# arangesh/Ground-Plane-Polling

Hardware: AMD Instinct MI355X
Metric: images/sec end-to-end (resnet50, 1k planes, 1242x375) (higher is better)
Workload: dtype f16x3

## Files before the change

ground-plane-polling_amd/csrc/decode.hip:

```cpp

#include <hip/hip_runtime.h>
#include <stdint.h>
#include <limits.h>

#include <atomic>
#include <mutex>
#include <vector>

#include "gpp.h"

namespace {

constexpr int kCounterStride = 4096;
constexpr int kHeaderBytes = 64 * kCounterStride;
constexpr int kKeptCountWord = 1;
constexpr int kKeptKeysOffset = 1024;

__device__ __forceinline__ float cephes_expf(float x)
{
    x = fminf(fmaxf(x, -88.3762626647949f), 88.3762626647949f);
    float fx = floorf(x * 1.44269504088896341f + 0.5f);
    x = (x - fx * 0.693359375f) - fx * -2.12194440e-4f;
    const float z = x * x;
    float y = 1.9875691500e-4f;
// ... 766 lines not shown
}

__global__ __launch_bounds__(kCompactThreads) void compact_pixels_kernel(uint32_t* __restrict__ bitmap, const LevelTable T, int B, int max_rows,
                                                                         int32_t* __restrict__ rows, int32_t* __restrict__ counts,
                                                                         int32_t* __restrict__ flag, const int32_t* __restrict__ or_flag)
{
    compact_pixels(bitmap, T, B, max_rows, rows, counts, flag, or_flag);
}

struct CompactJob { uint32_t* bitmap; int32_t* rows; int32_t* counts; int32_t* flag; const int32_t* or_flag; };
__global__ __launch_bounds__(kCompactThreads) void compact_pixels_pair_kernel(const CompactJob a, const CompactJob b, const CompactJob c, const LevelTable T,
                                                                              int B, int max_rows)
{
    const CompactJob& j = blockIdx.x == 0 ? a : blockIdx.x == 1 ? b : c;
    compact_pixels(j.bitmap, T, B, max_rows, j.rows, j.counts, j.flag, j.or_flag);
}

__global__ __launch_bounds__(256) void mark_candidate_pixels_kernel(const float* __restrict__ cls, int64_t n_anchors, int nba, float thr,
                                                                    const LevelTable T, int B, int total_words, uint32_t* __restrict__ marks)
{
    __shared__ unsigned long long hit[4];
    const int lane = threadIdx.x & 63, wave = threadIdx.x >> 6;
    const int64_t gbit0 = (int64_t)blockIdx.x * 256 + wave * 64;
    const int word0 = (int)(gbit0 >> 5);
    if (lane == 0) hit[wave] = 0;
    __syncthreads();
    for (int i = 0; i < nba; ++i) {
        const int j = i * 64 + lane, q = j / nba, k = j - q * nba;
        const int word = word0 + (q >> 5);
        if (word >= total_words) continue;
// ... 79 lines not shown
#pragma unroll
        for (int s = 32; s >= 1; s >>= 1) n[k] += __shfl_down(n[k], s, 64);
        if (lane == 0) sums[k][wave] = n[k];
    }
    __syncthreads();
    if (tid == 0) {
        int t[4] = {0, 0, 0, 0};
        for (int q = 0; q < kCompactThreads / 64; ++q) { t[0] += sums[0][q]; t[1] += sums[1][q]; t[2] += sums[2][q]; t[3] += sums[3][q]; }
        const int f3 = (t[0] > max_rows || t[1] > tower_max_rows) ? 1 : 0;
        const int f2 = (f3 || t[2] > deep_max_rows) ? 1 : 0;
        stats[0] = t[0];
        stats[1] = t[1];
        stats[2] = f3;
        stats[3] = f2;
        if (stats0 != nullptr) stats0[0] = (f2 || t[3] > deep_max_rows) ? 1 : 0;
    }
}

std::mutex g_deep_mutex;
std::vector<gpp_deep_list_desc> g_deep_descs;
std::vector<char> g_deep_held;

}

extern "C" int gpp_detect_pixel_lists(const gpp_pixel_list_desc* host_desc, void* stream)
{
    if (!host_desc) return GPP_ERR_BAD_ARG;
    const gpp_pixel_list_desc& d = *host_desc;
    if (d.B < 0 || d.B > kMaxBatch || d.n_anchors <= 0 || d.n_anchors > kMaxAnchors || d.num_base_anchors <= 0 || d.max_rows < 0 ||
        d.n_levels < 1 || d.n_levels > GPP_MAX_GROUPS || (d.lists_per_image != 1 && d.lists_per_image != 4) || d.reserved != 0 || d.reserved2 != 0)
// ... 45 lines not shown

int deep_lists_table(const gpp_deep_list_desc& d, LevelTable& T, int64_t& words)
{
    if (d.B < 0 || d.B > kMaxBatch || d.n_anchors <= 0 || d.n_anchors > kMaxAnchors || d.num_base_anchors <= 0 || d.num_base_anchors > 64 ||
        d.max_rows < 0 || d.tower_max_rows < 0 || d.deep_max_rows < 0 || d.n_levels < 1 || d.n_levels > GPP_MAX_GROUPS || d.reserved != 0 ||
        !(d.score_thr == d.score_thr))
        return GPP_ERR_BAD_ARG;
    const bool layer1 = d.rows1 || d.counts1 || d.flag1;
    const bool layer0 = d.radius4 || d.rows0 || d.counts0 || d.flag0 || d.stats0;
    if (layer0 && (!d.radius4 || !d.rows0 || !d.counts0 || !d.flag0 || !d.stats0 || !d.rows1 || !d.counts1 || !d.flag1)) return GPP_ERR_BAD_ARG;
    if (d.B > 0 && (!d.cls_logits || !d.marks || !d.radius1 || !d.radius2 || !d.radius3 || !d.rows2 || !d.counts2 || !d.flag2 || !d.stats ||
                    (layer1 && (!d.rows1 || !d.counts1 || !d.flag1))))
        return GPP_ERR_BAD_ARG;
    if (((uintptr_t)d.cls_logits & 15) || (((uintptr_t)d.marks | (uintptr_t)d.radius1 | (uintptr_t)d.radius2 | (uintptr_t)d.radius3 | (uintptr_t)d.rows2 |
          (uintptr_t)d.counts2 | (uintptr_t)d.flag2 | (uintptr_t)d.rows1 | (uintptr_t)d.counts1 | (uintptr_t)d.flag1 | (uintptr_t)d.stats |
          (uintptr_t)d.radius4 | (uintptr_t)d.rows0 | (uintptr_t)d.counts0 | (uintptr_t)d.flag0 | (uintptr_t)d.stats0) & 3))
        return GPP_ERR_ALIGN;
    T.n_levels = d.n_levels;
    int64_t pixels = 0;
    words = 0;
    for (int l = 0; l < GPP_MAX_GROUPS; ++l) {
        const int pix = l < d.n_levels ? d.level_pixels[l] : 0;
        if (l < d.n_levels && pix <= 0) return GPP_ERR_BAD_ARG;
        if ((int64_t)d.B * (pixels + pix) >= (1LL << 31)) return GPP_ERR_UNSUPPORTED;
        T.pix[l] = pix;
        T.pix_begin[l] = (int)pixels;
        T.word_begin[l] = (int)words;
        T.list_begin[l] = (int)((int64_t)d.B * pixels);
        T.width[l] = l < d.n_levels ? d.level_width[l] : 0;
        if (l < d.n_levels && (T.width[l] <= 0 || pix % T.width[l] != 0)) return GPP_ERR_BAD_ARG;
        pixels += pix;
        words += ((int64_t)d.B * pix + 31) / 32;
    }
    if (pixels * d.num_base_anchors != d.n_anchors) return GPP_ERR_BAD_ARG;
    return GPP_OK;
}

}

extern "C" int gpp_detect_deep_lists(const gpp_deep_list_desc* host_desc, void* stream)
{
    if (!host_desc) return GPP_ERR_BAD_ARG;
    const gpp_deep_list_desc& d = *host_desc;
    LevelTable T;
    int64_t words = 0;
    const int rc = deep_lists_table(d, T, words);
    if (rc != GPP_OK) return rc;
    if (d.B == 0) return GPP_OK;
    hipStream_t st = (hipStream_t)stream;
    const unsigned blocks = (unsigned)(((words + 1) / 2 * 64 + 255) / 256);
    mark_candidate_pixels_kernel<<<dim3(blocks), 256, 0, st>>>(d.cls_logits, d.n_anchors, d.num_base_anchors, d.score_thr, T, d.B, (int)words, d.marks);
    if (d.radius4) dilate_radii_kernel<true><<<dim3(blocks), 256, 0, st>>>(d.marks, T, d.B, (int)words, d.radius1, d.radius2, d.radius3, d.radius4);
    else dilate_radii_kernel<false><<<dim3(blocks), 256, 0, st>>>(d.marks, T, d.B, (int)words, d.radius1, d.radius2, d.radius3, nullptr);
    deep_stats_kernel<<<1, kCompactThreads, 0, st>>>(d.marks, d.radius1, d.radius2, (int)words, d.max_rows, d.tower_max_rows, d.deep_max_rows, d.stats,
                                                     d.radius3, d.stats0);
    const CompactJob layer2 = {d.radius2, d.rows2, d.counts2, d.flag2, d.stats + 2}, layer1 = {d.radius3, d.rows1, d.counts1, d.flag1, d.stats + 3};
    const CompactJob layer0 = {d.radius4, d.rows0, d.counts0, d.flag0, d.stats0};
    if (d.rows1) compact_pixels_pair_kernel<<<d.rows0 ? 3 : 2, kCompactThreads, 0, st>>>(layer2, layer1, layer0, T, d.B, d.deep_max_rows);
    else compact_pixels_kernel<<<1, kCompactThreads, 0, st>>>(d.radius2, T, d.B, d.deep_max_rows, d.rows2, d.counts2, d.flag2, d.stats + 2);
    const hipError_t e = hipGetLastError();
    return e == hipSuccess ? GPP_OK : (int)e;
}

extern "C" int gpp_detect_deep_lists_register(const gpp_deep_list_desc* host_desc, int32_t* handle)
{
    if (!host_desc || !handle) return GPP_ERR_BAD_ARG;
    LevelTable T;
    int64_t words = 0;
// ... 81 lines not shown
```

ground-plane-polling_amd/keras_retinanet_3D/backend/hip.py:

```python

import ctypes
import os

_LIB = None
_HERE = os.path.dirname(os.path.abspath(__file__))
LIB_PATH = os.environ.get('GPP_LIB') or os.path.normpath(os.path.join(_HERE, '..', '..', 'lib', 'libgpp_hip.so'))
CSRC_DIR = os.path.normpath(os.path.join(_HERE, '..', '..', 'csrc'))

GPP_OK = 0
_ERRORS = {
    -1: 'GPP_ERR_BAD_ARG',
    -2: 'GPP_ERR_WORKSPACE',
    -3: 'GPP_ERR_ALIGN',
    -4: 'GPP_ERR_UNSUPPORTED',
}

c_void_p = ctypes.c_void_p
c_int = ctypes.c_int
c_float = ctypes.c_float
c_size_t = ctypes.c_size_t
c_int64 = ctypes.c_int64


GPP_BF16 = 1
# ... 52 lines not shown
class PixelListDesc(ctypes.Structure):
    _fields_ = [('workspace', c_void_p), ('bitmap', c_void_p), ('rows', c_void_p), ('counts', c_void_p), ('flag', c_void_p),
                ('n_anchors', c_int64)] + \
               [(n, ctypes.c_int32) for n in ('B', 'num_base_anchors', 'lists_per_image', 'n_levels', 'max_rows', 'reserved')] + \
               [('level_pixels', ctypes.c_int32 * GPP_MAX_GROUPS), ('reserved2', ctypes.c_int32)] + \
               [('dilated_bitmap', c_void_p), ('dilated_rows', c_void_p), ('dilated_counts', c_void_p), ('dilated_flag', c_void_p),
                ('level_width', ctypes.c_int32 * GPP_MAX_GROUPS), ('dilated_max_rows', ctypes.c_int32)]


class DeepListDesc(ctypes.Structure):
    _fields_ = [(n, c_void_p) for n in ('cls_logits', 'marks', 'radius1', 'radius2', 'radius3', 'rows2', 'counts2', 'flag2',
                                        'rows1', 'counts1', 'flag1', 'stats')] + [('n_anchors', c_int64)] + \
               [(n, ctypes.c_int32) for n in ('B', 'num_base_anchors', 'n_levels', 'max_rows', 'tower_max_rows', 'deep_max_rows')] + \
               [('score_thr', c_float), ('reserved', ctypes.c_int32),
                ('level_pixels', ctypes.c_int32 * GPP_MAX_GROUPS), ('level_width', ctypes.c_int32 * GPP_MAX_GROUPS)] + \
               [(n, c_void_p) for n in ('radius4', 'rows0', 'counts0', 'flag0', 'stats0')]


class MobileNetBlockDesc(ctypes.Structure):
    _fields_ = [('inp', c_void_p), ('dw_weight', c_void_p), ('dw_bias', c_void_p), ('pw_weight', c_void_p), ('pw_bias', c_void_p),
                ('out_scale', c_void_p), ('out', c_void_p)] + \
               [(n, ctypes.c_int32) for n in ('dtype', 'B', 'H', 'W', 'C_in', 'C_out', 'stride', 'in_pitch', 'out_pitch', 'weight_rows',
                                              'tile_hint', 'reserved')]


class MobileNetStemDesc(ctypes.Structure):
    _fields_ = [('inp', c_void_p), ('weight', c_void_p), ('bias', c_void_p), ('out', c_void_p)] + \
               [(n, ctypes.c_int32) for n in ('B', 'H', 'W', 'C_out', 'out_pitch', 'reserved')]


class AbsmaxDesc(ctypes.Structure):
# ... 144 lines not shown
        lib.gpp_road_peel_workspace_bytes.argtypes = [c_int, c_int, ctypes.POINTER(c_size_t)]
        lib.gpp_road_peel_i32.restype = c_int
        lib.gpp_road_peel_i32.argtypes = [c_void_p] * 4 + [c_uint32, c_void_p] + [c_int] * 4 + [c_double] + [c_void_p] * 3 + [c_size_t, c_void_p]
    if hasattr(lib, 'gpp_detect_pixel_lists'):
        lib.gpp_detect_pixel_lists.restype = c_int
        lib.gpp_detect_pixel_lists.argtypes = [ctypes.POINTER(PixelListDesc), c_void_p]
    if hasattr(lib, 'gpp_detect_deep_lists'):
        lib.gpp_detect_deep_lists.restype = c_int
        lib.gpp_detect_deep_lists.argtypes = [ctypes.POINTER(DeepListDesc), c_void_p]
        lib.gpp_detect_deep_lists_register.restype = c_int
        lib.gpp_detect_deep_lists_register.argtypes = [ctypes.POINTER(DeepListDesc), ctypes.POINTER(ctypes.c_int32)]
        lib.gpp_detect_deep_lists_release.restype = c_int
        lib.gpp_detect_deep_lists_release.argtypes = [ctypes.c_int32]
        lib.gpp_detect_deep_lists_run.restype = c_int
        lib.gpp_detect_deep_lists_run.argtypes = [ctypes.c_int32, c_int, c_void_p]
    if hasattr(lib, 'gpp_conv2d_deferred_register'):
        lib.gpp_conv2d_deferred_register.restype = c_int
        lib.gpp_conv2d_deferred_register.argtypes = [ctypes.POINTER(ConvDesc), ctypes.POINTER(ctypes.c_int32)]
        lib.gpp_conv2d_deferred_release.restype = c_int
        lib.gpp_conv2d_deferred_release.argtypes = [ctypes.c_int32]
        lib.gpp_conv2d_deferred_run.restype = c_int
        lib.gpp_conv2d_deferred_run.argtypes = [ctypes.c_int32, c_int, c_void_p]
    lib.gpp_conv2d_igemm.restype = c_int
    lib.gpp_conv2d_igemm.argtypes = [ctypes.POINTER(ConvDesc), c_void_p]
    lib.gpp_stem_conv7x7_bn_relu.restype = c_int
    lib.gpp_stem_conv7x7_bn_relu.argtypes = [c_void_p, c_void_p, c_void_p, c_void_p, c_int, c_int, c_int, c_int, c_void_p]
    lib.gpp_stem_conv7x7_bn_relu_mfma.restype = c_int
    lib.gpp_stem_conv7x7_bn_relu_mfma.argtypes = [c_void_p, c_void_p, c_void_p, c_void_p, c_int, c_int, c_int, c_int, c_void_p]
    lib.gpp_stem_pack_weights_f16.restype = c_int
    lib.gpp_stem_pack_weights_f16.argtypes = [c_void_p, c_void_p, c_size_t]
# ... 694 lines not shown
```

ground-plane-polling_amd/keras_retinanet_3D/models/builder.py:

```python

import ctypes

from ..backend import hip
from ..layers import conv as C
from ..layers import mobilenet as M
from ..layers.filter_detections import MAX_DETECTIONS, NMS_THRESHOLD, SCORE_THRESHOLD
from ..utils import anchors as anchor_utils
from ..utils import cuboid_nms as cuboid_nms_utils
from ..utils.gpp_utils import POLL_THRESHOLD, POSE_SCORE_THRESHOLD
from . import weights as W
from .plan import (BlockDesc, BlockProjDesc, CandidatePixelsDesc, CuboidNmsDesc, DensePoolDesc, DetectDesc, PollDesc, PoolDesc, PoseDesc,
                   PreactDesc, RaggedPoolDesc, RaggedStemDesc, ReluDesc, StemDesc, TailDesc,
                   OP_STEM, OP_MAXPOOL, OP_CONV, OP_RELU, OP_DETECT, OP_POLL, OP_TAIL, OP_BLOCK,
                   OP_DETECT_CANDIDATES, OP_DETECT_SELECT, OP_DETECT_EMIT, OP_DETECT_OSF, OP_STEM_POOL,
                   OP_MAXPOOL_PAD, OP_AVGPOOL, OP_CONV_PREACT, OP_MOBILENET_STEM, OP_MOBILENET_BLOCK, OP_POSE, OP_CUBOID_NMS,
                   OP_ABSMAX, OP_ABSMAX_CLEAR, OP_STEM_RAGGED, OP_STEM_POOL_RAGGED, OP_MAXPOOL_RAGGED, OP_DETECT_CANDIDATE_PIXELS,
                   block_form, head_forms, layer_split, part_of, TOWER_SLICES, TOWER0, TOWER0_SLICE, SparseHeads, Plan)


class PlanBuilder(object):

    def __init__(self, model, B, H, Wd, n_planes, planes_batched, ragged=False):
        torch, dev = model.torch, model.device
        self.model, self.torch, self.device = model, torch, dev
# ... 346 lines not shown
            plan.keep += plan.sparse.tensors()
            if forms.deep_layers:
                plan.sparse.add_deep(self.torch, forms.deep_layers, opts.sparse_deep)
                plan.keep += plan.sparse.deep_tensors()
            if forms.tower0:
                plan.sparse.add_tower0(self.torch)
                plan.keep += plan.sparse.tower0_tensors()
        if forms.tower0:
            self.towers_0_split(P, wide)
        else:
            self.conv(TOWER0, P, wide, 3, pad=(1, 1), relu=True, join=True)
        l_dim, l_cls = (1, 2) if opts.head_lanes else (0, 0)
        towers = {'cls': ('pyramid_classification', 256, 512, 'pyramid_classification', cls_o, 0, l_cls or opts.cls_lane),
                  'reg': ('pyramid_regression', 512, 0, 'pyramid_regression_ops', reg_o, 1, 0, bool(opts.cls_lane)),
                  'dim': ('pyramid_regression_dim', 128, 768, 'pyramid_regression_dim', dim_o, 0, l_dim)}
        if opts.decode_overlap:
            self.tower(forms, wide, *towers['cls'])
            self.decode(OP_DETECT_CANDIDATE_PIXELS if plan.sparse else OP_DETECT_CANDIDATES, 'filtered_detections/candidates',
                        lane=opts.cls_lane or 1)
            self.tower(forms, wide, *towers['reg'])
            self.decode(OP_DETECT_SELECT, 'filtered_detections/select', lane=1, sync=True)
            self.tower(forms, wide, *towers['dim'])
            self.decode(OP_DETECT_EMIT, join=True)
        else:
            for t in ('dim', 'cls', 'reg'):
                self.tower(forms, wide, *towers[t])
            self.decode(OP_DETECT_OSF if m.osf else OP_DETECT, join=True)

    def towers_0_split(self, P, wide):
        m, plan, sp = self.model, self.plan, self.plan.sparse
        wt, bias, (kh, kw, cin, cout) = m.conv_w[TOWER0]
# ... 10 lines not shown
                            out_scale=parts[2] if scale is not None else None)
            if m.dtype == 'f16x3':
                d.range_counter = plan.range_slot.data_ptr()
            return d
        rest = desc(n, cout - n)
        plan.conv_descs.append((rest, 0))
        plan.ws_need[0] = max(plan.ws_need.get(0, 0), C.workspace_bytes(rest))
        first = desc(0, n)
        first.weight_rows = n
        first.deep_rows, first.deep_counts, first.deep_flag = sp.tower0_rows.data_ptr(), sp.tower0_counts.data_ptr(), sp.tower0_flag.data_ptr()
        plan.keep.append(first)
        plan.emit(OP_CONV, rest, TOWER0, list(P), cols(n, cout - n), flops=C.conv_flops(rest) + C.conv_flops(first), join=True, io=(P, wide, None))
        self.tower0 = (first, list(P), cols(0, n))

    def tower(self, forms, wide, prefix, width, c0, out_name, out, tag=0, lane=0, join=False):
        src = [C.FMap(f.buf, f.B, f.H, f.W, width, off=f.off + c0, bstride=f.bstride, pitch=f.pitch, split=f.split, half=f.half) for f in wide]
        regression = out_name == 'pyramid_regression_ops'
        for i in range(1, 4):
            name = '{}_{}'.format(prefix, i)
            _, dst = self.pyramid(width)
            if regression and i == 3 and forms.tower_both:
                self.tower_last(name, src, dst, tag, lane)
            elif regression and 3 - forms.deep_layers <= i < 3:
                self.tower_deep(name, src, dst, tag, lane, 2 - i)
            else:
                self.conv(name, src, dst, 3, pad=(1, 1), relu=True, tag=tag, lane=lane)
            src = dst
        self.out_layer('dense' if lane else forms.outputs[out_name], out_name, src, out, lane, join)

    def tower_last(self, name, src, dst, tag, lane):
        sp = self.plan.sparse
        d = self.desc(name, src, dst, 3, pad=(1, 1), relu=True, lane=lane)
        d.tower_rows, d.tower_counts, d.tower_flag = sp.tower_rows.data_ptr(), sp.tower_counts.data_ptr(), sp.tower_flag.data_ptr()
        self.plan.emit(OP_CONV, d, name, list(src) + [sp.tower_rows, sp.tower_counts, sp.tower_flag], dst, tag=tag, flops=C.conv_flops(d), lane=lane,
                       join=not sp.lists_joined, io=(src, dst, None))
        sp.lists_joined = True
        sp.tower.append(d)

    def tower_deep(self, name, src, dst, tag, lane, which):
        sp = self.plan.sparse
        d = self.desc(name, src, dst, 3, pad=(1, 1), relu=True, lane=lane)
        lists = [sp.deep_rows[which], sp.deep_counts[which], sp.deep_flags[which]]
        d.deep_rows, d.deep_counts, d.deep_flag = [t.data_ptr() for t in lists]
        self.plan.emit(OP_CONV, d, name, list(src) + lists, dst, tag=tag, flops=C.conv_flops(d), lane=lane, io=(src, dst, None))
        sp.deep.append(d)

    def out_layer(self, form, name, src, out, lane, join):
        plan, sp = self.plan, self.plan.sparse
        if form == 'lists_after':
            d = self.desc(name, src, out, 3, pad=(1, 1), out_f32=True, lane=lane)
            d.lists_after = sp.register_deep(sp.deep_desc(plan.cls_logits, plan.n_anchors, anchor_utils.NUM_BASE_ANCHORS, SCORE_THRESHOLD))
            reads, writes = list(src), list(out) + sp.deep_tensors()
            if sp.tower0_rows is not None:
                first, p_maps, slice_maps = self.tower0
                sp.register_tower0(first, d)
                reads, writes = reads + p_maps, writes + slice_maps + sp.tower0_tensors()
            plan.emit(OP_CONV, d, name, reads, writes, flops=C.conv_flops(d), lane=lane, join=join, io=(src, out, None))
            return
        if form == 'dense':
            self.conv(name, src, out, 3, pad=(1, 1), out_f32=True, lane=lane, join=join)
            if sp is not None and join and not lane:
                sp.lists_joined = True
            return
        dense = self.desc(name, src, out, 3, pad=(1, 1), out_f32=True, lane=lane)
        dense.guard, dense.guard_value = sp.flag.data_ptr(), 1
        plan.emit(OP_CONV, dense, name, list(src) + [sp.flag], out, flops=C.conv_flops(dense), lane=lane, join=join or not sp.lists_joined,
                  io=(src, out, None))
        sp.lists_joined = True
        rows = self.desc(name, src, out, 3, pad=(1, 1), out_f32=True, lane=lane)
        rows.gather_rows, rows.gather_counts, rows.split_k = sp.rows.data_ptr(), sp.counts.data_ptr(), 1
        rows.guard, rows.guard_value = sp.flag.data_ptr(), 0
        plan.emit(OP_CONV, rows, name, list(src) + [sp.rows, sp.counts, sp.flag], out, lane=lane, io=(src, out, None))
        sp.dense.append(dense)
        sp.gathered.append(rows)

    def poll(self):
        plan, B, n_planes, torch, dev, D = self.plan, self.B, self.n_planes, self.torch, self.device, MAX_DETECTIONS
        plan.keypoints = torch.empty((B, D, 4, 3), dtype=torch.float32, device=dev)
# ... 118 lines not shown
```

ground-plane-polling_amd/keras_retinanet_3D/models/plan.py:

```python

import collections
import ctypes
import os

import numpy as np

from ..backend import hip
from ..layers import conv as C


class StemDesc(ctypes.Structure):
    _fields_ = [('inp', ctypes.c_void_p), ('weight', ctypes.c_void_p), ('bias', ctypes.c_void_p), ('out', ctypes.c_void_p),
                ('dtype', ctypes.c_int32), ('B', ctypes.c_int32), ('H', ctypes.c_int32), ('W', ctypes.c_int32), ('range_counter', ctypes.c_void_p)]


class PoolDesc(ctypes.Structure):
    _fields_ = [('inp', ctypes.c_void_p), ('out', ctypes.c_void_p), ('dtype', ctypes.c_int32), ('B', ctypes.c_int32),
                ('H', ctypes.c_int32), ('W', ctypes.c_int32), ('C', ctypes.c_int32), ('reserved', ctypes.c_int32)]


class RaggedStemDesc(ctypes.Structure):
    _fields_ = [('stem', StemDesc), ('heights', ctypes.c_void_p), ('Hp', ctypes.c_int32), ('reserved', ctypes.c_int32)]


# ... 69 lines not shown
OP_STEM_POOL = 13
OP_MAXPOOL_PAD, OP_AVGPOOL, OP_CONV_PREACT = 17, 18, 32
OP_MOBILENET_STEM, OP_MOBILENET_BLOCK = 33, 34
OP_POSE = 19
OP_CUBOID_NMS = 20
OP_ABSMAX, OP_ABSMAX_CLEAR = 35, 36
OP_STEM_RAGGED, OP_STEM_POOL_RAGGED, OP_MAXPOOL_RAGGED = 37, 38, 39
OP_DETECT_CANDIDATE_PIXELS = 40
DETECT_OPS = (OP_DETECT, OP_DETECT_CANDIDATES, OP_DETECT_SELECT, OP_DETECT_EMIT, 12, OP_DETECT_CANDIDATE_PIXELS)
OP_JOIN, OP_SYNC = 0x10000, 0x20000


PlanOptions = collections.namedtuple('PlanOptions', 'x3_level fuse_stem_pool stage_chunks half_stages fuse_tail fuse_block fuse_block_proj '
                                                    'fuse_block_inproj fuse_inproj_rounds '
                                                    'br1_lane fpn_lanes p4_lane head_lanes decode_overlap cls_lane autotune tune_key sparse_heads '
                                                    'sparse_tower sparse_tower_rounds sparse_deep sparse_deep_rounds sparse_depth')


def plan_options(model, B):
    env = os.environ.get
    x3 = model.dtype in C.X3_TYPES
    x3_split = env('GPP_X3_SPLIT', '2')
    x3_level = int(x3_split) if x3 else 0
    chunks = env('GPP_STAGE_CHUNKS')
    tail_widths = env('GPP_FUSE_TAIL', '64,128')
    fuse_tail = [int(v) for v in tail_widths.split(',') if v.strip() and int(v) > 0]
    if x3:
        fuse_tail = [v for v in fuse_tail if v == 64] if x3_level >= 2 else []
    elif model.esz == 4:
        fuse_tail = []
    block_widths = env('GPP_FUSE_BLOCK', '64,128')
# ... 17 lines not shown
        fuse_inproj_rounds=float(env('GPP_FUSE_INPROJ_MIN_ROUNDS', FUSE_INPROJ_MIN_ROUNDS)),
        br1_lane=env('GPP_BR1_LANE', '1') != '0',
        fpn_lanes=fpn_lanes,
        p4_lane=1 if (fpn_lanes and env('GPP_P4_LANE', '1') != '0') else 0,
        head_lanes=head_lanes,
        decode_overlap=overlap,
        cls_lane=2 if (overlap and env('GPP_CLS_LANE', '1' if B <= 2 else '0') != '0') else 0,
        autotune=env('GPP_AUTOTUNE', '1') != '0',
        sparse_heads=max(1e-9, float(env('GPP_SPARSE_HEADS_MAX_SHARE', SPARSE_HEADS_MAX_SHARE))) if sparse else 0.0,
        sparse_tower=(max(1e-9, float(env('GPP_SPARSE_TOWER_MAX_SHARE', SPARSE_TOWER_MAX_SHARE)))
                      if (sparse and env('GPP_SPARSE_TOWER', '1') != '0') else 0.0),
        sparse_tower_rounds=float(env('GPP_SPARSE_TOWER_MIN_ROUNDS', SPARSE_TOWER_MIN_ROUNDS)),
        sparse_deep=max(1e-9, float(env('GPP_SPARSE_TOWER_DEEP_MAX_SHARE', SPARSE_TOWER_DEEP_MAX_SHARE))),
        sparse_deep_rounds=float(env('GPP_SPARSE_TOWER_DEEP_MIN_ROUNDS', SPARSE_TOWER_DEEP_MIN_ROUNDS)),
        sparse_depth=int(env('GPP_SPARSE_TOWER_DEPTH', SPARSE_TOWER_DEPTH)),
        tune_key='x3split={};fuse={}/{};plan={}{}'.format(x3_split, tail_widths, block_widths, model.plan_mode,
                                                          C.latency_split_config() if model.plan_mode == 'latency' else '') +
                 (';audit' if model.audit else '') + ('' if inproj else ';inproj=0'))


INPROJ_TILE = (8, 14)
FUSE_INPROJ_MIN_ROUNDS = '1'


def inproj_rounds(images, h, w):
    th, tw = INPROJ_TILE
    return images * (-(-h // th)) * (-(-w // tw)) / (2.0 * COMPUTE_UNITS)


def block_form(opts, width, projection, split_input, halves, join, inproj=None):
    if (projection and inproj is not None and opts.fuse_block_inproj and width == 64 and width in opts.fuse_block and inproj[0] == 1 and
            inproj_rounds(*inproj[1:]) > opts.fuse_inproj_rounds):
        return 'block', 'inproj'
# ... 103 lines not shown
        self.flag = torch.ones((1,), dtype=i32, device=device)
        self.dense, self.gathered = [], []
        self.lists_joined = False
        self.tower, self.tower_max_rows = [], 0
        self.tower_bitmap = self.tower_rows = self.tower_counts = self.tower_flag = self.range_scratch = None
        if tower_share > 0.0:
            self.tower_max_rows = max(0, min(total, int(tower_share * total)))
            self.tower_bitmap = torch.zeros_like(self.bitmap)
            self.tower_rows = torch.zeros_like(self.rows)
            self.tower_counts = torch.zeros_like(self.counts)
            self.tower_flag = torch.ones_like(self.flag)
            self.range_scratch = torch.zeros((1,), dtype=torch.int64, device=device)

        self.deep, self.deep_layers, self.deep_max_rows, self.deep_handle = [], 0, 0, 0
        self.deep_bitmaps = self.deep_rows = self.deep_counts = self.deep_flags = self.deep_stats = None
        self.tower0 = self.tower0_carrier = None
        self.tower0_handle = 0
        self.tower0_bitmap = self.tower0_rows = self.tower0_counts = self.tower0_flag = self.tower0_stats = None

    def add_tower0(self, torch):
        self.tower0_bitmap = torch.zeros_like(self.bitmap)
        self.tower0_rows = torch.zeros_like(self.rows)
        self.tower0_counts = torch.zeros_like(self.counts)
        self.tower0_flag = torch.ones_like(self.flag)
        self.tower0_stats = torch.zeros_like(self.flag)

    def tower0_tensors(self):
        if self.tower0_rows is None:
            return []
        return [self.tower0_bitmap, self.tower0_rows, self.tower0_counts, self.tower0_flag, self.tower0_stats]
# ... 25 lines not shown
    def deep_desc(self, cls_logits, n_anchors, num_base_anchors, score_thr):
        d = hip.DeepListDesc()
        d.cls_logits = cls_logits.data_ptr()
        d.marks, d.radius1, d.radius2, d.radius3 = [t.data_ptr() for t in self.deep_bitmaps]
        d.rows2, d.counts2, d.flag2 = self.deep_rows[0].data_ptr(), self.deep_counts[0].data_ptr(), self.deep_flags[0].data_ptr()
        if self.deep_layers > 1:
            d.rows1, d.counts1, d.flag1 = self.deep_rows[1].data_ptr(), self.deep_counts[1].data_ptr(), self.deep_flags[1].data_ptr()
        d.stats = self.deep_stats.data_ptr()
        if self.tower0_rows is not None:
            d.radius4, d.rows0, d.counts0 = self.tower0_bitmap.data_ptr(), self.tower0_rows.data_ptr(), self.tower0_counts.data_ptr()
            d.flag0, d.stats0 = self.tower0_flag.data_ptr(), self.tower0_stats.data_ptr()
        d.n_anchors, d.B, d.num_base_anchors, d.n_levels = n_anchors, self.B, num_base_anchors, len(self.level_pixels)
        d.max_rows, d.tower_max_rows, d.deep_max_rows, d.score_thr = self.max_rows, self.tower_max_rows, self.deep_max_rows, score_thr
        d.level_pixels = (ctypes.c_int32 * hip.GPP_MAX_GROUPS)(*self.level_pixels)
        d.level_width = (ctypes.c_int32 * hip.GPP_MAX_GROUPS)(*self.level_widths)
        return d

    def register_deep(self, desc):
        handle = ctypes.c_int32(0)
        hip.check(hip.lib().gpp_detect_deep_lists_register(ctypes.byref(desc), ctypes.byref(handle)), 'gpp_detect_deep_lists_register')
        self.deep_handle = int(handle.value)
        return self.deep_handle

    def __del__(self):
        if getattr(self, 'deep_handle', 0):
            try:
                hip.lib().gpp_detect_deep_lists_release(self.deep_handle)
            except Exception:
                pass
            self.deep_handle = 0
# ... 31 lines not shown
        for flag in list(self.deep_flags or ()) + ([self.tower0_flag] if self.tower0_flag is not None else []):
            flag.fill_(1)


class Plan(object):

    def __init__(self):
        self.keep = []
        self.io = {}
        self.io_parts = {}
        self.tuning_parts = {}
        self.ops = []
        self.oracle_names = {}
        self.lanes = []
        self.access = []
        self.atomic = []
        self.wrote = []
        self.op_io = []
        self.audit_table = None
        self.audit_maps = []
        self.audit_unobserved = []
        self.inner = {}
        self.open_lanes = set()
        self.conv_descs = []
        self.ws_need = {}
        self.array = None
        self.flops = 0.0
        self.ragged = False
        self.heights = None
        self.sparse = None
        self.heads_stale = False

    @property
    def regression(self):
        self.complete_heads()
        return self._regression

    @regression.setter
# ... 24 lines not shown
                    setattr(d, field, None)
                setattr(d, tile, 0)
                if scratch and d.range_counter:
                    d.range_counter = sp.range_scratch.data_ptr()
                if sp.tower0 is not None and desc is sp.deep[0]:
                    d.conv_before = sp.tower0_handle
                hip.check(hip.lib().gpp_conv2d_igemm(ctypes.byref(d), hip.stream_ptr()), 'gpp_conv2d_igemm ({})'.format(what))

    def emit(self, kind, desc, name, reads=(), writes=(), tag=0, flops=0.0, lane=0, join=False, sync=False, io=None, inner=(), atomic=()):
        self.keep += list(inner) + [desc]
        if inner:
            self.inner[id(desc)] = tuple(inner)
        self.ops.append((kind, tag, desc, name, flops))
        self.lanes.append((int(lane) << 8) | (OP_JOIN if join else 0) | (OP_SYNC if sync else 0))
        self.access.append((self.spans(reads), self.spans(writes)))
        self.atomic.append(self.spans(atomic))
        self.wrote.append([x for x in writes if isinstance(x, C.FMap)])
        self.op_io.append(io)
        self.flops += flops
        if lane:
            self.open_lanes.add(lane)
        elif join:
            self.open_lanes.clear()
        if io is not None:
            self.io[name] = io
            self.io_parts.setdefault(name, []).append(io)

    @staticmethod
    def span(fm):
        e = fm.buf.element_size()
# ... 13 lines not shown
        old = (self.ops, self.lanes, self.access, self.atomic, self.wrote, self.op_io)
        self.ops, self.lanes, self.access, self.atomic, self.wrote, self.op_io = [], [], [], [], [], []
        for pos, row in enumerate(zip(*old)):
            for dst, item in zip((self.ops, self.lanes, self.access, self.atomic, self.wrote, self.op_io), row):
                dst.append(item)
            for kind, desc, name, reads, atomic in extra.get(pos, ()):
                self.keep.append(desc)
                self.ops.append((kind, 0, desc, name, 0.0))
                self.lanes.append(row[1] & 0xff00)
                self.access.append((self.spans(reads), []))
                self.atomic.append(self.spans(atomic))
                self.wrote.append([])
                self.op_io.append(None)

    def check_stream_ordering(self):
        def overlap(a, b):
            return any(x0 < y1 and y0 < x1 for x0, x1 in a for y0, y1 in b)
        bad, seen = [], []
        active = {}
        forks, joins = {}, []
        for pos, (kind, _, desc, name, _) in enumerate(self.ops):
            flags = self.lanes[pos]
            lane, join, sync = (flags >> 8) & 0xff, bool(flags & OP_JOIN), bool(flags & OP_SYNC)
            if lane > 0:
                if not active.get(lane) or sync:
                    forks.setdefault(lane, []).append(pos)
                    active[lane] = True
            elif join:
                joins.append(pos)
                active = {}
            reads, writes = self.access[pos]
            atomic = self.atomic[pos]
# ... 42 lines not shown
```

include/gpp.h:

```cpp
#ifndef GPP_H_
#define GPP_H_

#include <stddef.h>
#include <stdint.h>

#ifdef __cplusplus
extern "C" {
#endif

#define GPP_OK 0
#define GPP_ERR_BAD_ARG (-1)
#define GPP_ERR_WORKSPACE (-2)
#define GPP_ERR_ALIGN (-3)
#define GPP_ERR_UNSUPPORTED (-4)

const char* gpp_version(void);

int gpp_poll_workspace_bytes(int B, int N, int planes_batched, size_t* bytes);

int gpp_poll_f32(const float* boxes, const float* dims, const int32_t* orient, const float* P_inv,
                 const float* planes, int B, int D, int N, int planes_batched, float thr,
                 float* keypoints, float* keyplanes, float* residuals, int32_t* best_idx,
                 void* workspace, size_t workspace_bytes, void* stream);

// ... 177 lines not shown
    int32_t level_width[GPP_MAX_GROUPS]; int32_t dilated_max_rows;
} gpp_pixel_list_desc;
int gpp_detect_pixel_lists(const gpp_pixel_list_desc* host_desc, void* stream);

typedef struct gpp_deep_list_desc {
    const float* cls_logits;
    uint32_t* marks; uint32_t* radius1; uint32_t* radius2; uint32_t* radius3;
    int32_t* rows2; int32_t* counts2; int32_t* flag2;
    int32_t* rows1; int32_t* counts1; int32_t* flag1;
    int32_t* stats;
    int64_t n_anchors;
    int32_t B, num_base_anchors, n_levels, max_rows, tower_max_rows, deep_max_rows;
    float score_thr; int32_t reserved;
    int32_t level_pixels[GPP_MAX_GROUPS]; int32_t level_width[GPP_MAX_GROUPS];
    uint32_t* radius4; int32_t* rows0; int32_t* counts0; int32_t* flag0; int32_t* stats0;
} gpp_deep_list_desc;
int gpp_detect_deep_lists(const gpp_deep_list_desc* host_desc, void* stream);
int gpp_detect_deep_lists_register(const gpp_deep_list_desc* host_desc, int32_t* handle);
int gpp_detect_deep_lists_release(int32_t handle);
int gpp_detect_deep_lists_run(int32_t handle, int check_only, void* stream);

int gpp_detect_osf_workspace_bytes(int B, int64_t n_anchors, size_t* bytes);
int gpp_detect_osf_f32(const float* cls_logits, const float* regression, const float* regression_dim,
                       const float* anchors, int B, int64_t n_anchors, int num_base_anchors, int fused_layout,
                       float score_thr, float iou_thr, int max_det,
                       float* boxes, float* dims, float* scores, int32_t* labels, int32_t* orientations,
                       int32_t* anchor_index, int32_t* counts,
                       void* workspace, size_t workspace_bytes, void* stream);

int gpp_pack_detections(const float* boxes, const float* dims, const float* scores, const int32_t* labels,
                        const int32_t* orientations, const float* keypoints, const float* keyplanes,
                        const float* residuals, int B, int D, float* packed, void* stream);
// ... 291 lines not shown
```

Before: 946.1.

## Parallelize deep-list compaction into per-chunk workgroups with precomputed prefix bases

Replaces the single-workgroup-per-map pixel compaction for the deep sparse tower lists with a two-pass scheme. A stats kernel popcounts each 64-word chunk and scans them into per-chunk base offsets, and a grid of chunk workgroups then scatters row indices in parallel. This needs a new scratch buffer allocated from the Python plan. It also adds an opt-in dim-tower side lane (off by default) and a column-aware overlap check in the stream-ordering validator. The goal is to remove the serial bottleneck of one-block compaction, at the cost of an extra launch and scratch memory.

```diff
diff --git a/ground-plane-polling_amd/csrc/decode.hip b/ground-plane-polling_amd/csrc/decode.hip
--- a/ground-plane-polling_amd/csrc/decode.hip
+++ b/ground-plane-polling_amd/csrc/decode.hip
@@ -804,6 +804,48 @@
 {
     const CompactJob& j = blockIdx.x == 0 ? a : blockIdx.x == 1 ? b : c;
     compact_pixels(j.bitmap, T, B, max_rows, j.rows, j.counts, j.flag, j.or_flag);
+}
+
+struct ChunkTable { int n_maps; int chunk_begin[GPP_MAX_GROUPS + 1]; };
+constexpr int kChunkThreads = GPP_DEEP_CHUNK_WORDS * 4;
+static_assert(kChunkThreads % 64 == 0 && kChunkThreads <= 1024, "whole wavefronts, one workgroup");
+__device__ __forceinline__ int chunk_level(const ChunkTable& K, int n_levels, int chunk)
+{
+    int l = 0;
+    for (int q = 1; q < n_levels; ++q) l = chunk >= K.chunk_begin[q] ? q : l;
+    return l;
+}
+__global__ __launch_bounds__(kChunkThreads) void compact_chunks_kernel(const CompactJob a, const CompactJob b, const CompactJob c, const LevelTable T,
+                                                                       const ChunkTable K, int B, const int32_t* bases)
+{
+    __shared__ int wave_sum[kChunkThreads / 64];
+    const CompactJob& j = blockIdx.y == 0 ? a : blockIdx.y == 1 ? b : c;
+    const int tid = threadIdx.x, lane = tid & 63, wave = tid >> 6, chunk = blockIdx.x;
+    const int l = chunk_level(K, T.n_levels, chunk);
+    const int n_words = (B * T.pix[l] + 31) >> 5;
+    const int w = (chunk - K.chunk_begin[l]) * GPP_DEEP_CHUNK_WORDS + (tid >> 2), shift = (tid & 3) * 8;
+    uint32_t* slot = j.bitmap + T.word_begin[l] + w;
+    const uint32_t word = w < n_words ? *slot : 0u;
+    uint32_t byte = (word >> shift) & 0xffu;
+    const int n = __popc(byte);
+    int incl = n;
+#pragma unroll
+    for (int s = 1; s < 64; s <<= 1) {
+        const int up = __shfl_up(incl, s, 64);
+        if (lane >= s) incl += up;
+    }
+    if (lane == 63) wave_sum[wave] = incl;
+    __syncthreads();
+    int before = 0;
+#pragma unroll
+    for (int q = 0; q < kChunkThreads / 64; ++q) before += q < wave ? wave_sum[q] : 0;
+    if (shift == 0 && word) *slot = 0;
+    int pos = bases[(int64_t)blockIdx.y * K.chunk_begin[GPP_MAX_GROUPS] + chunk] + before + incl - n;
+    while (byte) {
+        const int bit = __ffs((int)byte) - 1;
+        byte &= byte - 1;
+        j.rows[T.list_begin[l] + pos++] = w * 32 + shift + bit;
+    }
 }
 
 __global__ __launch_bounds__(256) void mark_candidate_pixels_kernel(const float* __restrict__ cls, int64_t n_anchors, int nba, float thr,
@@ -913,6 +955,94 @@
         stats[2] = f3;
         stats[3] = f2;
         if (stats0 != nullptr) stats0[0] = (f2 || t[3] > deep_max_rows) ? 1 : 0;
+    }
+}
+
+__global__ __launch_bounds__(kCompactThreads) void deep_stats_chunks_kernel(const uint32_t* __restrict__ marks, const uint32_t* __restrict__ radius1,
+                                                                            int total_words, int max_rows, int tower_max_rows, int deep_max_rows,
+                                                                            int32_t* __restrict__ stats, int32_t* __restrict__ stats0,
+                                                                            const CompactJob a, const CompactJob b, const CompactJob c,
+                                                                            const LevelTable T, const ChunkTable K, int B, int32_t* bases)
+{
+    constexpr int kWaves = kCompactThreads / 64;
+    __shared__ int sums[2][kWaves];
+    __shared__ int level_count[3][GPP_MAX_GROUPS];
+    const int tid = threadIdx.x, lane = tid & 63, wave = tid >> 6;
+    int n[2] = {0, 0};
+    for (int w = tid; w < total_words; w += kCompactThreads) {
+        n[0] += __popc(marks[w]);
+        n[1] += __popc(radius1[w]);
+    }
+#pragma unroll
+    for (int k = 0; k < 2; ++k) {
+#pragma unroll
+        for (int s = 32; s >= 1; s >>= 1) n[k] += __shfl_down(n[k], s, 64);
+        if (lane == 0) sums[k][wave] = n[k];
+    }
+    constexpr int kSlots = 8;
+    const int n_chunks = K.chunk_begin[GPP_MAX_GROUPS], n_slots = K.n_maps * n_chunks;
+    for (int i0 = wave; i0 < n_slots; i0 += kWaves * kSlots) {
+        int bits[kSlots];
+#pragma unroll
+        for (int u = 0; u < kSlots; ++u) {
+            const int i = min(i0 + u * kWaves, n_slots - 1);
+            const int m = i >= 2 * n_chunks ? 2 : i >= n_chunks ? 1 : 0, chunk = i - m * n_chunks;
+            const int l = chunk_level(K, T.n_levels, chunk);
+            const int n_words = (B * T.pix[l] + 31) >> 5;
+            const int w = (chunk - K.chunk_begin[l]) * GPP_DEEP_CHUNK_WORDS + lane;
+            const uint32_t* map = m == 0 ? a.bitmap : m == 1 ? b.bitmap : c.bitmap;
+            const uint32_t word = map[T.word_begin[l] + min(w, n_words - 1)];
+            bits[u] = w < n_words ? __popc(word) : 0;
+        }
+#pragma unroll
+        for (int s = 32; s >= 1; s >>= 1) {
+#pragma unroll
+            for (int u = 0; u < kSlots; ++u) bits[u] += __shfl_down(bits[u], s, 64);
+        }
+#pragma unroll
+        for (int u = 0; u < kSlots; ++u)
+            if (lane == 0 && i0 + u * kWaves < n_slots) bases[i0 + u * kWaves] = bits[u];
+    }
+    __syncthreads();
+    for (int i = wave; i < K.n_maps * GPP_MAX_GROUPS; i += kWaves) {
+        const int m = i / GPP_MAX_GROUPS, l = i - m * GPP_MAX_GROUPS;
+        int32_t* slots = bases + (int64_t)m * n_chunks;
+        int running = 0;
+        for (int c0 = K.chunk_begin[l]; c0 < K.chunk_begin[l + 1]; c0 += 64) {
+            const int k = c0 + lane;
+            const int v = k < K.chunk_begin[l + 1] ? slots[k] : 0;
+            int incl = v;
+#pragma unroll
+            for (int s = 1; s < 64; s <<= 1) {
+                const int up = __shfl_up(incl, s, 64);
+                if (lane >= s) incl += up;
+            }
+            if (k < K.chunk_begin[l + 1]) slots[k] = running + incl - v;
+            running += __shfl(incl, 63, 64);
+        }
+        if (lane == 0) level_count[m][l] = running;
+    }
+    __syncthreads();
+    if (tid == 0) {
+        int t[2] = {0, 0};
+        for (int q = 0; q < kWaves; ++q) { t[0] += sums[0][q]; t[1] += sums[1][q]; }
+        int or_flag = (t[0] > max_rows || t[1] > tower_max_rows) ? 1 : 0;
+        stats[0] = t[0];
+        stats[1] = t[1];
+        stats[2] = or_flag;
+        for (int m = 0; m < K.n_maps; ++m) {
+            const CompactJob& j = m == 0 ? a : m == 1 ? b : c;
+            int total = 0;
+            for (int l = 0; l < GPP_MAX_GROUPS; ++l) {
+                j.counts[l] = level_count[m][l];
+                total += level_count[m][l];
+            }
+            j.counts[GPP_MAX_GROUPS] = total;
+            or_flag = (total > deep_max_rows || or_flag) ? 1 : 0;
+            j.flag[0] = or_flag;
+            if (m == 0) stats[3] = or_flag;
+            if (m == 1 && stats0 != nullptr) stats0[0] = or_flag;
+        }
     }
 }
 
@@ -988,7 +1118,7 @@
         return GPP_ERR_BAD_ARG;
     if (((uintptr_t)d.cls_logits & 15) || (((uintptr_t)d.marks | (uintptr_t)d.radius1 | (uintptr_t)d.radius2 | (uintptr_t)d.radius3 | (uintptr_t)d.rows2 |
           (uintptr_t)d.counts2 | (uintptr_t)d.flag2 | (uintptr_t)d.rows1 | (uintptr_t)d.counts1 | (uintptr_t)d.flag1 | (uintptr_t)d.stats |
-          (uintptr_t)d.radius4 | (uintptr_t)d.rows0 | (uintptr_t)d.counts0 | (uintptr_t)d.flag0 | (uintptr_t)d.stats0) & 3))
+          (uintptr_t)d.radius4 | (uintptr_t)d.rows0 | (uintptr_t)d.counts0 | (uintptr_t)d.flag0 | (uintptr_t)d.stats0 | (uintptr_t)d.chunk_bases) & 3))
         return GPP_ERR_ALIGN;
     T.n_levels = d.n_levels;
     int64_t pixels = 0;
@@ -1010,6 +1140,29 @@
     return GPP_OK;
 }
 
+void deep_chunk_table(const LevelTable& T, int B, int n_maps, ChunkTable& K)
+{
+    K.n_maps = n_maps;
+    int chunks = 0;
+    for (int l = 0; l <= GPP_MAX_GROUPS; ++l) {
+        K.chunk_begin[l] = chunks;
+        if (l < T.n_levels) chunks += (int)((((int64_t)B * T.pix[l] + 31) / 32 + GPP_DEEP_CHUNK_WORDS - 1) / GPP_DEEP_CHUNK_WORDS);
+    }
+}
+
+}
+
+extern "C" int gpp_detect_deep_lists_scratch_bytes(const gpp_deep_list_desc* host_desc, size_t* bytes)
+{
+    if (!host_desc || !bytes) return GPP_ERR_BAD_ARG;
+    LevelTable T;
+    int64_t words = 0;
+    const int rc = deep_lists_table(*host_desc, T, words);
+    if (rc != GPP_OK) return rc;
+    ChunkTable K;
+    deep_chunk_table(T, host_desc->B, 3, K);
+    *bytes = (size_t)3 * (size_t)K.chunk_begin[GPP_MAX_GROUPS] * sizeof(int32_t);
+    return GPP_OK;
 }
 
 extern "C" int gpp_detect_deep_lists(const gpp_deep_list_desc* host_desc, void* stream)
@@ -1026,6 +1179,18 @@
     mark_candidate_pixels_kernel<<<dim3(blocks), 256, 0, st>>>(d.cls_logits, d.n_anchors, d.num_base_anchors, d.score_thr, T, d.B, (int)words, d.marks);
     if (d.radius4) dilate_radii_kernel<true><<<dim3(blocks), 256, 0, st>>>(d.marks, T, d.B, (int)words, d.radius1, d.radius2, d.radius3, d.radius4);
     else dilate_radii_kernel<false><<<dim3(blocks), 256, 0, st>>>(d.marks, T, d.B, (int)words, d.radius1, d.radius2, d.radius3, nullptr);
+    if (d.chunk_bases) {
+        const CompactJob layer2 = {d.radius2, d.rows2, d.counts2, d.flag2, nullptr}, layer1 = {d.radius3, d.rows1, d.counts1, d.flag1, nullptr};
+        const CompactJob layer0 = {d.radius4, d.rows0, d.counts0, d.flag0, nullptr};
+        ChunkTable K;
+        deep_chunk_table(T, d.B, d.rows0 ? 3 : d.rows1 ? 2 : 1, K);
+        deep_stats_chunks_kernel<<<1, kCompactThreads, 0, st>>>(d.marks, d.radius1, (int)words, d.max_rows, d.tower_max_rows, d.deep_max_rows, d.stats,
+                                                                d.stats0, layer2, layer1, layer0, T, K, d.B, d.chunk_bases);
+        compact_chunks_kernel<<<dim3((unsigned)K.chunk_begin[GPP_MAX_GROUPS], (unsigned)K.n_maps), kChunkThreads, 0, st>>>(layer2, layer1, layer0, T, K,
+                                                                                                                        d.B, d.chunk_bases);
+        const hipError_t e = hipGetLastError();
+        return e == hipSuccess ? GPP_OK : (int)e;
+    }
     deep_stats_kernel<<<1, kCompactThreads, 0, st>>>(d.marks, d.radius1, d.radius2, (int)words, d.max_rows, d.tower_max_rows, d.deep_max_rows, d.stats,
                                                      d.radius3, d.stats0);
     const CompactJob layer2 = {d.radius2, d.rows2, d.counts2, d.flag2, d.stats + 2}, layer1 = {d.radius3, d.rows1, d.counts1, d.flag1, d.stats + 3};
diff --git a/ground-plane-polling_amd/keras_retinanet_3D/backend/hip.py b/ground-plane-polling_amd/keras_retinanet_3D/backend/hip.py
--- a/ground-plane-polling_amd/keras_retinanet_3D/backend/hip.py
+++ b/ground-plane-polling_amd/keras_retinanet_3D/backend/hip.py
@@ -90,7 +90,10 @@
                [(n, ctypes.c_int32) for n in ('B', 'num_base_anchors', 'n_levels', 'max_rows', 'tower_max_rows', 'deep_max_rows')] + \
                [('score_thr', c_float), ('reserved', ctypes.c_int32),
                 ('level_pixels', ctypes.c_int32 * GPP_MAX_GROUPS), ('level_width', ctypes.c_int32 * GPP_MAX_GROUPS)] + \
-               [(n, c_void_p) for n in ('radius4', 'rows0', 'counts0', 'flag0', 'stats0')]
+               [(n, c_void_p) for n in ('radius4', 'rows0', 'counts0', 'flag0', 'stats0', 'chunk_bases')]
+
+
+GPP_DEEP_CHUNK_WORDS = 64
 
 
 class MobileNetBlockDesc(ctypes.Structure):
@@ -265,6 +268,9 @@
         lib.gpp_detect_deep_lists_release.argtypes = [ctypes.c_int32]
         lib.gpp_detect_deep_lists_run.restype = c_int
         lib.gpp_detect_deep_lists_run.argtypes = [ctypes.c_int32, c_int, c_void_p]
+    if hasattr(lib, 'gpp_detect_deep_lists_scratch_bytes'):
+        lib.gpp_detect_deep_lists_scratch_bytes.restype = c_int
+        lib.gpp_detect_deep_lists_scratch_bytes.argtypes = [ctypes.POINTER(DeepListDesc), ctypes.POINTER(c_size_t)]
     if hasattr(lib, 'gpp_conv2d_deferred_register'):
         lib.gpp_conv2d_deferred_register.restype = c_int
         lib.gpp_conv2d_deferred_register.argtypes = [ctypes.POINTER(ConvDesc), ctypes.POINTER(ctypes.c_int32)]
diff --git a/ground-plane-polling_amd/keras_retinanet_3D/models/builder.py b/ground-plane-polling_amd/keras_retinanet_3D/models/builder.py
--- a/ground-plane-polling_amd/keras_retinanet_3D/models/builder.py
+++ b/ground-plane-polling_amd/keras_retinanet_3D/models/builder.py
@@ -384,7 +384,21 @@
         towers = {'cls': ('pyramid_classification', 256, 512, 'pyramid_classification', cls_o, 0, l_cls or opts.cls_lane),
                   'reg': ('pyramid_regression', 512, 0, 'pyramid_regression_ops', reg_o, 1, 0, bool(opts.cls_lane)),
                   'dim': ('pyramid_regression_dim', 128, 768, 'pyramid_regression_dim', dim_o, 0, l_dim)}
-        if opts.decode_overlap:
+        plan.dim_lane = opts.dim_lane if (forms.tower0 and self.B >= 2 and opts.decode_overlap and not opts.cls_lane and not opts.head_lanes and
+                                          not m.audit and m.plan_mode != 'latency') else 0
+        if plan.dim_lane:
+            cls, reg = self.tower_steps(forms, wide, *towers['cls']), self.tower_steps(forms, wide, *towers['reg'])
+            dim = self.tower_steps(forms, wide, *towers['dim'][:-1], lane=plan.dim_lane, sync=(1, 2), side_form=True)
+            for step in cls[:3] + dim[:1] + cls[3:]:
+                step()
+            self.decode(OP_DETECT_CANDIDATE_PIXELS, 'filtered_detections/candidates', lane=1)
+            for step in reg[:3] + dim[1:2] + reg[3:]:
+                step()
+            self.decode(OP_DETECT_SELECT, 'filtered_detections/select', lane=1, sync=True)
+            for step in dim[2:]:
+                step()
+            self.decode(OP_DETECT_EMIT, join=True)
+        elif opts.decode_overlap:
             self.tower(forms, wide, *towers['cls'])
             self.decode(OP_DETECT_CANDIDATE_PIXELS if plan.sparse else OP_DETECT_CANDIDATES, 'filtered_detections/candidates',
                         lane=opts.cls_lane or 1)
@@ -425,19 +439,27 @@
         self.tower0 = (first, list(P), cols(0, n))
 
     def tower(self, forms, wide, prefix, width, c0, out_name, out, tag=0, lane=0, join=False):
-        src = [C.FMap(f.buf, f.B, f.H, f.W, width, off=f.off + c0, bstride=f.bstride, pitch=f.pitch, split=f.split, half=f.half) for f in wide]
+        for step in self.tower_steps(forms, wide, prefix, width, c0, out_name, out, tag, lane, join):
+            step()
+
+    def tower_steps(self, forms, wide, prefix, width, c0, out_name, out, tag=0, lane=0, join=False, sync=(), side_form=False):
+        maps = [[C.FMap(f.buf, f.B, f.H, f.W, width, off=f.off + c0, bstride=f.bstride, pitch=f.pitch, split=f.split, half=f.half) for f in wide]]
         regression = out_name == 'pyramid_regression_ops'
-        for i in range(1, 4):
-            name = '{}_{}'.format(prefix, i)
+
+        def layer(i):
+            name, src = '{}_{}'.format(prefix, i), maps[-1]
             _, dst = self.pyramid(width)
             if regression and i == 3 and forms.tower_both:
                 self.tower_last(name, src, dst, tag, lane)
             elif regression and 3 - forms.deep_layers <= i < 3:
                 self.tower_deep(name, src, dst, tag, lane, 2 - i)
             else:
-                self.conv(name, src, dst, 3, pad=(1, 1), relu=True, tag=tag, lane=lane)
-            src = dst
-        self.out_layer('dense' if lane else forms.outputs[out_name], out_name, src, out, lane, join)
+                self.conv(name, src, dst, 3, pad=(1, 1), relu=True, tag=tag, lane=lane, sync=i in sync)
+            maps.append(dst)
+
+        def output():
+            self.out_layer(forms.outputs[out_name] if (side_form or not lane) else 'dense', out_name, maps[-1], out, lane, join)
+        return [lambda: layer(1), lambda: layer(2), lambda: layer(3), output]
 
     def tower_last(self, name, src, dst, tag, lane):
         sp = self.plan.sparse
@@ -461,7 +483,7 @@
         if form == 'lists_after':
             d = self.desc(name, src, out, 3, pad=(1, 1), out_f32=True, lane=lane)
             d.lists_after = sp.register_deep(sp.deep_desc(plan.cls_logits, plan.n_anchors, anchor_utils.NUM_BASE_ANCHORS, SCORE_THRESHOLD))
-            reads, writes = list(src), list(out) + sp.deep_tensors()
+            reads, writes = list(src), list(out) + sp.deep_tensors() + ([sp.deep_scratch] if sp.deep_scratch is not None else [])
             if sp.tower0_rows is not None:
                 first, p_maps, slice_maps = self.tower0
                 sp.register_tower0(first, d)
@@ -473,6 +495,8 @@
             if sp is not None and join and not lane:
                 sp.lists_joined = True
             return
+        if lane and not sp.lists_joined:
+            raise ValueError('{}: a gathered output layer on side lane {} needs the lists joined in front of its fork'.format(name, lane))
         dense = self.desc(name, src, out, 3, pad=(1, 1), out_f32=True, lane=lane)
         dense.guard, dense.guard_value = sp.flag.data_ptr(), 1
         plan.emit(OP_CONV, dense, name, list(src) + [sp.flag], out, flops=C.conv_flops(dense), lane=lane, join=join or not sp.lists_joined,
diff --git a/ground-plane-polling_amd/keras_retinanet_3D/models/plan.py b/ground-plane-polling_amd/keras_retinanet_3D/models/plan.py
--- a/ground-plane-polling_amd/keras_retinanet_3D/models/plan.py
+++ b/ground-plane-polling_amd/keras_retinanet_3D/models/plan.py
@@ -107,7 +107,7 @@
 PlanOptions = collections.namedtuple('PlanOptions', 'x3_level fuse_stem_pool stage_chunks half_stages fuse_tail fuse_block fuse_block_proj '
                                                     'fuse_block_inproj fuse_inproj_rounds '
                                                     'br1_lane fpn_lanes p4_lane head_lanes decode_overlap cls_lane autotune tune_key sparse_heads '
-                                                    'sparse_tower sparse_tower_rounds sparse_deep sparse_deep_rounds sparse_depth')
+                                                    'sparse_tower sparse_tower_rounds sparse_deep sparse_deep_rounds sparse_depth dim_lane')
 
 
 def plan_options(model, B):
@@ -155,9 +155,14 @@
         sparse_deep=max(1e-9, float(env('GPP_SPARSE_TOWER_DEEP_MAX_SHARE', SPARSE_TOWER_DEEP_MAX_SHARE))),
         sparse_deep_rounds=float(env('GPP_SPARSE_TOWER_DEEP_MIN_ROUNDS', SPARSE_TOWER_DEEP_MIN_ROUNDS)),
         sparse_depth=int(env('GPP_SPARSE_TOWER_DEPTH', SPARSE_TOWER_DEPTH)),
+        dim_lane=DIM_LANE if env('GPP_DIM_LANE', DIM_LANE_DEFAULT) != '0' else 0,
         tune_key='x3split={};fuse={}/{};plan={}{}'.format(x3_split, tail_widths, block_widths, model.plan_mode,
                                                           C.latency_split_config() if model.plan_mode == 'latency' else '') +
                  (';audit' if model.audit else '') + ('' if inproj else ';inproj=0'))
+
+
+DIM_LANE = 2
+DIM_LANE_DEFAULT = '0'
 
 
 INPROJ_TILE = (8, 14)
@@ -291,6 +296,7 @@
 
         self.deep, self.deep_layers, self.deep_max_rows, self.deep_handle = [], 0, 0, 0
         self.deep_bitmaps = self.deep_rows = self.deep_counts = self.deep_flags = self.deep_stats = None
+        self.deep_scratch = None
         self.tower0 = self.tower0_carrier = None
         self.tower0_handle = 0
         self.tower0_bitmap = self.tower0_rows = self.tower0_counts = self.tower0_flag = self.tower0_stats = None
@@ -346,6 +352,11 @@
         d.max_rows, d.tower_max_rows, d.deep_max_rows, d.score_thr = self.max_rows, self.tower_max_rows, self.deep_max_rows, score_thr
         d.level_pixels = (ctypes.c_int32 * hip.GPP_MAX_GROUPS)(*self.level_pixels)
         d.level_width = (ctypes.c_int32 * hip.GPP_MAX_GROUPS)(*self.level_widths)
+        if hasattr(hip.lib(), 'gpp_detect_deep_lists_scratch_bytes'):
+            need = hip.c_size_t(0)
+            hip.check(hip.lib().gpp_detect_deep_lists_scratch_bytes(ctypes.byref(d), ctypes.byref(need)), 'gpp_detect_deep_lists_scratch_bytes')
+            self.deep_scratch = self.rows.new_zeros((max(1, int(need.value) // 4),))
+            d.chunk_bases = self.deep_scratch.data_ptr()
         return d
 
     def register_deep(self, desc):
@@ -407,6 +418,7 @@
         self.oracle_names = {}
         self.lanes = []
         self.access = []
+        self.columns = {}
         self.atomic = []
         self.wrote = []
         self.op_io = []
@@ -415,6 +427,7 @@
         self.audit_unobserved = []
         self.inner = {}
         self.open_lanes = set()
+        self.dim_lane = 0
         self.conv_descs = []
         self.ws_need = {}
         self.array = None
@@ -469,6 +482,11 @@
         self.ops.append((kind, tag, desc, name, flops))
         self.lanes.append((int(lane) << 8) | (OP_JOIN if join else 0) | (OP_SYNC if sync else 0))
         self.access.append((self.spans(reads), self.spans(writes)))
+        for fm in [x for x in list(reads) + list(writes) if isinstance(x, C.FMap) and x.C < x.pitch]:
+            e = fm.buf.element_size()
+            for lo, hi in self.span(fm):
+                cols = (fm.buf.data_ptr(), fm.pitch * e, (lo - fm.buf.data_ptr()) % (fm.pitch * e), fm.C * e)
+                self.columns[(lo, hi)] = cols if self.columns.get((lo, hi), cols) == cols else None
         self.atomic.append(self.spans(atomic))
         self.wrote.append([x for x in writes if isinstance(x, C.FMap)])
         self.op_io.append(io)
@@ -512,8 +530,14 @@
                 self.op_io.append(None)
 
     def check_stream_ordering(self):
+        def apart(x, y):
+            p, q = self.columns.get(x), self.columns.get(y)
+            if p is None or q is None or p[:2] != q[:2] or p[2] + p[3] > p[1] or q[2] + q[3] > q[1]:
+                return False
+            return p[2] + p[3] <= q[2] or q[2] + q[3] <= p[2]
+
         def overlap(a, b):
-            return any(x0 < y1 and y0 < x1 for x0, x1 in a for y0, y1 in b)
+            return any(x0 < y1 and y0 < x1 and not apart((x0, x1), (y0, y1)) for x0, x1 in a for y0, y1 in b)
         bad, seen = [], []
         active = {}
         forks, joins = {}, []
diff --git a/include/gpp.h b/include/gpp.h
--- a/include/gpp.h
+++ b/include/gpp.h
@@ -215,8 +215,11 @@
     float score_thr; int32_t reserved;
     int32_t level_pixels[GPP_MAX_GROUPS]; int32_t level_width[GPP_MAX_GROUPS];
     uint32_t* radius4; int32_t* rows0; int32_t* counts0; int32_t* flag0; int32_t* stats0;
+    int32_t* chunk_bases;
 } gpp_deep_list_desc;
+#define GPP_DEEP_CHUNK_WORDS 64
 int gpp_detect_deep_lists(const gpp_deep_list_desc* host_desc, void* stream);
+int gpp_detect_deep_lists_scratch_bytes(const gpp_deep_list_desc* host_desc, size_t* bytes);
 int gpp_detect_deep_lists_register(const gpp_deep_list_desc* host_desc, int32_t* handle);
 int gpp_detect_deep_lists_release(int32_t handle);
 int gpp_detect_deep_lists_run(int32_t handle, int check_only, void* stream);
```

Result: no change. 942.6 (-0.4%).
